# BurnhamG/PyTorch-ScalableFHVAE

Measured on AMD Instinct MI355X. Metric: segments/sec + ELBO (nats/frame), (B,20,80) fbank, higher is better.
Workload: dtype bf16; 1 GPU; c3: fhvae.FHVAE 2x256 LSTM enc/dec, z1=z2=32, 28k-seq mu2 table, batch 2048; per-GPU batch 2048, T=20, F=80, full train step (fwd+loss+bwd+Adam), intended objective, mu_idx uniform; global_batch=2048, parallelism=single

## Files before the change

pytorch-scalablefhvae_amd/csrc/lstm_fwd_wr.hip:

```cpp
#include <cstdlib>
#include <type_traits>

#include "lstm_cluster_dev.h"

#include "trace.h"

namespace fh {

constexpr int kFwH = 256, kFwG = 4 * kFwH, kFwHU = 32, kFwNU = 8, kFwThreads = 512;
typedef void __attribute__((address_space(3))) * fw_lds_p;

template <int NP>
__device__ __forceinline__ void fw_h_offsets(unsigned (&voff)[NP], int r0, int rlast, int piece0, int lane) {
#pragma unroll
  for (int i = 0; i < NP; ++i) {
    const int rw = (piece0 + i) * 2 + (lane >> 5), rg = r0 + rw;
    voff[i] = (unsigned)(rg < rlast ? rg : rlast) * (kFwH * 2) + (unsigned)(((lane & 31) ^ (rw & 15)) << 4);
  }
}
template <int NP>
__device__ __forceinline__ void fw_dma_h(char* img, __amdgpu_buffer_rsrc_t rs, const unsigned (&voff)[NP], unsigned slab_bytes, int piece0) {
#pragma unroll
  for (int i = 0; i < NP; ++i)
    __builtin_amdgcn_raw_ptr_buffer_load_lds(rs, (fw_lds_p)(img + (piece0 + i) * 1024), 16, voff[i], slab_bytes, 0, kSc1);
}
template <int NP>
__device__ __forceinline__ void fw_x_offsets(unsigned (&voff)[NP], int I, int r0, int rlast, int piece0, int lane) {
#pragma unroll
  for (int i = 0; i < NP; ++i) {
    const int rw = (piece0 + i) * 4 + (lane >> 4), rg = r0 + rw;
    voff[i] = (unsigned)(rg < rlast ? rg : rlast) * (unsigned)(I * 2) + (unsigned)(((lane & 15) ^ (rw & 15)) << 4);
  }
}
template <int NP>
__device__ __forceinline__ void fw_dma_x(char* img, __amdgpu_buffer_rsrc_t rs, const unsigned (&voff)[NP], unsigned slab_bytes, int nchx, int piece0,
                                         int lane) {
#pragma unroll
  for (int i = 0; i < NP; ++i) {
    const int rw = (piece0 + i) * 4 + (lane >> 4);
    if (((lane & 15) ^ (rw & 15)) < nchx)
      __builtin_amdgcn_raw_ptr_buffer_load_lds(rs, (fw_lds_p)(img + (piece0 + i) * 1024), 16, voff[i], slab_bytes, 0, 0);
  }
}
template <int NP>
__device__ __forceinline__ void fw_dma_xc(char* img, const u16* xc, int Ic, const u16* pad, int nchx, int r0, int rlast, int piece0, int lane) {
  const int nchc = Ic >> 3;
#pragma unroll
  for (int i = 0; i < NP; ++i) {
    const int rw = (piece0 + i) * 4 + (lane >> 4), rg = r0 + rw;
    const int64_t rc = rg < rlast ? rg : rlast;
    const int c = (lane & 15) ^ (rw & 15);
    if (c >= nchx) {
      const u16* src = c < nchx + nchc ? xc + rc * Ic + (c - nchx) * 8 : pad;
      __builtin_amdgcn_global_load_lds((const void __attribute__((address_space(1)))*)src, (fw_lds_p)(img + (piece0 + i) * 1024), 16, 0, 0);
    }
  }
}

template <int RT, int PDT = 4>
__global__ __launch_bounds__(kFwThreads) void lstm_fwd_wr_kernel(ClFwd p) {
  constexpr bool kSave = true;
#include "lstm_fwd_wr_body.h"
}
template <int RT, int PDT = 4>
__global__ __launch_bounds__(kFwThreads) void lstm_fwd_wr_infer_kernel(ClFwd p) {
  constexpr bool kSave = false;
#include "lstm_fwd_wr_body.h"
}

template __global__ void lstm_fwd_wr_kernel<2>(ClFwd);
template __global__ void lstm_fwd_wr_kernel<4>(ClFwd);
template __global__ void lstm_fwd_wr_infer_kernel<2>(ClFwd);
template __global__ void lstm_fwd_wr_infer_kernel<4>(ClFwd);

int cluster_fwd_wr(const ClFwd& p, hipStream_t st) {
  if ((int64_t)2 * p.T * p.B * kFwH * 2 >= (1LL << 31) || (int64_t)p.T * p.B * p.I * 2 >= (1LL << 31)) return FHVAE_ERR_LIMIT;
  if (p.NU != kFwNU || p.Mc > 64 || p.Mc % 16 != 0 || p.pre || p.K0 != p.I + p.Ic || p.K0 <= 0 || p.K0 > 128 || (p.I % 8) || (p.Ic % 8) ||
      (p.I > 0 && !p.x) || (p.Ic > 0 && !p.xcv))
    return FHVAE_ERR_SHAPE;
  const bool save = p.gates != nullptr;
  if (p.Mc <= 32 && save)
    hipLaunchKernelGGL((lstm_fwd_wr_kernel<2>), dim3(kGrid), dim3(kFwThreads), 0, st, p);
  else if (save)
    hipLaunchKernelGGL((lstm_fwd_wr_kernel<4>), dim3(kGrid), dim3(kFwThreads), 0, st, p);
  else if (p.Mc <= 32)
    hipLaunchKernelGGL((lstm_fwd_wr_infer_kernel<2>), dim3(kGrid), dim3(kFwThreads), 0, st, p);
  else
    hipLaunchKernelGGL((lstm_fwd_wr_infer_kernel<4>), dim3(kGrid), dim3(kFwThreads), 0, st, p);
  return fh_launch_status();
}

}
```

pytorch-scalablefhvae_amd/csrc/lstm_fwd_wr_body.h:

```cpp
  constexpr int H = kFwH, G = kFwG;
  constexpr int ROWS = RT * 16;
  __shared__ __attribute__((aligned(1024))) char img_h0[ROWS * 512];
  __shared__ __attribute__((aligned(1024))) char img_x[ROWS * 256];
  __shared__ __attribute__((aligned(1024))) char img_h1[ROWS * 512];
  constexpr int kGS = 272, kCS = 144, kHS = 80;
  constexpr int kStageL = ROWS * (kGS + 2 * kCS);
  __shared__ __attribute__((aligned(16))) char stage_all[2 * kStageL];
  __shared__ __attribute__((aligned(16))) char h16_all[ROWS * kHS];
  __shared__ int misc[2];
  const int tid = threadIdx.x, lane = tid & 63, wave = tid >> 6;
  const int r = lane & 15, q = lane >> 4;

  const int joined = cluster_join(p.sync, misc);
  if (joined < 0) return;
  const int info = joined & 255;
  const unsigned ep0 = (unsigned)(joined >> 8) * kSeqEpochs;
  const int cluster = (info >> 5) * (32 / kFwNU) + (info & 31) / kFwNU, me = (info & 31) % kFwNU;
  const int r0 = p.row0 + cluster * p.Mc;
  const int rend = min(p.row0 + p.nrows, r0 + p.Mc);
  if (r0 >= rend) return;
  unsigned* flags = p.sync + kSyncFlags + cluster * 32;
  unsigned* flagsB = flags + 8;
  const int B = p.B, T = p.T;
  const int um = me * kFwHU;
  const int ul = wave * 4 + q;
  if (tid == 0) misc[1] = 0;
  const int wv = __builtin_amdgcn_readfirstlane(wave);
  __syncthreads();

  const int wrow = (r & 3) * H + um + wave * 4 + (r >> 2);
  bf16x8 w_hh0[8], w_ih1[8], w_hh1[8], w_x[4];
#pragma unroll
  for (int ks = 0; ks < 8; ++ks) {
    const int64_t o = (int64_t)wrow * H + ks * 32 + q * 8;
    w_hh0[ks] = __builtin_bit_cast(bf16x8, *(const uint4*)(p.w_hh[0] + o));
    w_ih1[ks] = __builtin_bit_cast(bf16x8, *(const uint4*)(p.w_ih[1] + o));
    w_hh1[ks] = __builtin_bit_cast(bf16x8, *(const uint4*)(p.w_hh[1] + o));
  }
  const int nch0 = p.K0 / 8, nkx = (p.K0 + 31) / 32;
#pragma unroll
  for (int j = 0; j < 4; ++j) {
    const int c = j * 4 + q;
    uint4 v = uint4{0u, 0u, 0u, 0u};
    if (c < nch0) v = *(const uint4*)(p.w_ih0 + (int64_t)wrow * p.K0 + c * 8);
    w_x[j] = __builtin_bit_cast(bf16x8, v);
  }
  f32x4 add0, add1;
#pragma unroll
  for (int g = 0; g < 4; ++g) {
    add0[g] = p.b_ih[0][g * H + um + ul] + p.b_hh[0][g * H + um + ul];
    add1[g] = p.b_ih[1][g * H + um + ul] + p.b_hh[1][g * H + um + ul];
  }
  int hbase[4], xbase[4];
#pragma unroll
  for (int k3 = 0; k3 < 4; ++k3) {
    hbase[k3] = r * 512 + (((k3 * 4 + q) ^ r) << 4);
    xbase[k3] = r * 256 + (((k3 * 4 + q) ^ r) << 4);
  }
  float creg[2][RT];
#pragma unroll
  for (int l = 0; l < 2; ++l)
#pragma unroll
    for (int rt = 0; rt < RT; ++rt) creg[l][rt] = 0.f;
  unsigned long long* tl = (p.tlog && cluster == 0 && me == 0) ? p.tlog : nullptr;
  const bool xvar = p.I > 0;
  constexpr int NPX = RT * 4 / 4, NPH = RT * 8 / 4;
  const int nchx = p.I >> 3;
  const __amdgpu_buffer_rsrc_t hs_rs = make_rsrc(p.hs);
  const __amdgpu_buffer_rsrc_t x_rs = make_rsrc(xvar ? p.x : p.hs);
  unsigned voff_h[NPH], voff_x[NPX];
  fw_h_offsets<NPH>(voff_h, r0, rend - 1, (wv & 3) * NPH, lane);
  fw_x_offsets<NPX>(voff_x, p.I, r0, rend - 1, (wv & 3) * NPX, lane);
  const unsigned slab_h = (unsigned)B * (kFwH * 2), slab_x = (unsigned)B * (unsigned)(p.I * 2);
  if (wv < 4) {
    fw_dma_xc<NPX>(img_x, p.xcv, p.Ic, xvar ? p.x : p.xcv, nchx, r0, rend - 1, wv * NPX, lane);
    if (xvar) fw_dma_x<NPX>(img_x, x_rs, voff_x, 0u, nchx, wv * NPX, lane);
  }

  auto tail_stores = [&](int sp, int l, int wbase) {
    if (wv < wbase || wv >= wbase + 4) return;
    const int tq = tid - wbase * 64;
    const int t = sp - l;
    if (t < 0 || t >= T) return;
    const int64_t lt = (int64_t)l * T + t;
    const char* st = stage_all + l * kStageL;
    if constexpr (kSave) {
#pragma unroll
      for (int i = 0; i < ROWS * 16 / 256; ++i) {
        const int c = i * 256 + tq, rw = c >> 4, part = c & 15;
        const uint4 v = *(const uint4*)(st + rw * kGS + part * 16);
        if (r0 + rw < rend) *(uint4*)(p.gates + (lt * B + r0 + rw) * G + um * 4 + part * 8) = v;
      }
    }
    const bool top = l == 1 && p.hs_top_f32, last = p.hn && t == T - 1;
#pragma unroll
    for (int i = 0; i < ROWS * 8 / 256; ++i) {
      const int c = i * 256 + tq, rw = c >> 3, part = c & 7;
      if constexpr (kSave) {
        const uint4 v = *(const uint4*)(st + ROWS * kGS + rw * kCS + part * 16);
        if (r0 + rw < rend) *(uint4*)(p.cs + (lt * B + r0 + rw) * H + um + part * 4) = v;
      }
      if (top || last) {
        const uint4 hv = *(const uint4*)(st + ROWS * (kGS + kCS) + rw * kCS + part * 16);
        if (r0 + rw < rend) {
          if (top) *(uint4*)(p.hs_top_f32 + ((int64_t)t * B + r0 + rw) * H + um + part * 4) = hv;
          if (last) {
            *(uint4*)(p.hn + (int64_t)(r0 + rw) * (2 * H) + l * H + um + part * 4) = hv;
            if (p.hn_lp) {
              const float4 hf = __builtin_bit_cast(float4, hv);
              *(uint2*)(p.hn_lp + (int64_t)(r0 + rw) * (2 * H) + l * H + um + part * 4) = pack4(f32x4{hf.x, hf.y, hf.z, hf.w});
            }
          }
        }
      }
    }
  };
  auto h_out = [&](int l, int t, unsigned* fl, unsigned epoch, bool publish) {
    asm volatile("s_waitcnt lgkmcnt(0)\n\ts_barrier" ::: "memory");
    if (tid < ROWS * 4) {
      const int rw = tid >> 2, part = tid & 3;
      const uint4 v = *(const uint4*)(h16_all + rw * kHS + part * 16);
      if (r0 + rw < rend) *(uint4*)(p.hs + (((int64_t)l * T + t) * B + r0 + rw) * H + um + part * 8) = v;
    }
    if (publish) {
      if (wv < 4) asm volatile("s_waitcnt vmcnt(0)" ::: "memory");
      __syncthreads();
      if (tid == 0) __hip_atomic_store(fl + me, epoch, RLX_AGENT);
    } else {
      __syncthreads();
    }
  };
  auto flags_peek = [&](const unsigned* fl) -> unsigned {
    unsigned v = 0xffffffffu;
    if (lane < kFwNU) v = __hip_atomic_load(fl + lane, RLX_AGENT);
    return v;
  };
  auto flags_ready = [&](unsigned peeked, const unsigned* fl, unsigned epoch) -> bool {
    if (__all(peeked >= epoch)) return true;
    return cluster_wait(p.sync, fl, kFwNU, epoch);
  };
  unsigned peekA = 0u, peekB = 0u;

  constexpr int NI = 8 * RT;
  for (int s = 0; s <= T; ++s) {
    CL_TLOG(s * 8 + 0);
    const bool act0 = s < T, act1 = s >= 1;
    f32x4 acc[2][RT];
#pragma unroll
    for (int l = 0; l < 2; ++l)
#pragma unroll
      for (int rt = 0; rt < RT; ++rt) acc[l][rt] = f32x4{0.f, 0.f, 0.f, 0.f};
    if (wv < 4) asm volatile("s_waitcnt vmcnt(0)" ::: "memory");
    asm volatile("s_barrier" ::: "memory");
    if (misc[1]) return;
    CL_TLOG(s * 8 + 1);
    if (wv >= 4 && s >= 2) peekB = flags_peek(flagsB);
    if (s > 0) tail_stores(s - 1, 1, 0);
    auto mm = [&](auto l_c, const char* img, const bf16x8 (&w)[8], bool peek_a = false) {
      constexpr int l = decltype(l_c)::value;
      constexpr int PD = PDT;
      bf16x8 fb[PD + 1];
      auto frag = [&](int i) {
        const int ks = i / RT, rt = i % RT;
        fb[i % (PD + 1)] = __builtin_bit_cast(bf16x8, *(const uint4*)(img + hbase[ks & 3] + (ks >> 2) * 256 + rt * 8192));
      };
#pragma unroll
      for (int i = 0; i < PD; ++i) frag(i);
      if (PD > 2) __builtin_amdgcn_sched_barrier(0);
#pragma unroll
      for (int i = 0; i < NI; ++i) {
        const int ks = i / RT, rt = i % RT;
        if (i + PD < NI) frag(i + PD);
        if (PD > 2) __builtin_amdgcn_sched_barrier(0);
        acc[l][rt] = __builtin_amdgcn_mfma_f32_16x16x32_bf16(w[ks], fb[i % (PD + 1)], acc[l][rt], 0, 0, 0);
        if (PD > 2) __builtin_amdgcn_sched_barrier(0);
        if (i == NI - 1 && peek_a) peekA = flags_peek(flags);
      }
    };
    if (act0) {
#pragma unroll
      for (int j = 0; j < 4; ++j) {
        if (j >= nkx) break;
        bf16x8 b[RT];
#pragma unroll
        for (int rt = 0; rt < RT; ++rt) b[rt] = __builtin_bit_cast(bf16x8, *(const uint4*)(img_x + xbase[j] + rt * 4096));
        __builtin_amdgcn_sched_barrier(0);
#pragma unroll
        for (int rt = 0; rt < RT; ++rt) acc[0][rt] = __builtin_amdgcn_mfma_f32_16x16x32_bf16(w_x[j], b[rt], acc[0][rt], 0, 0, 0);
        __builtin_amdgcn_sched_barrier(0);
      }
      if (s > 0) mm(std::integral_constant<int, 0>{}, img_h0, w_hh0);
    }
    if (wv >= 4 && s >= 2) {
      if (!flags_ready(peekB, flagsB, ep0 + (unsigned)(s - 1))) {
        if (lane == 0) misc[1] = 1;
      } else {
        fw_dma_h<NPH>(img_h1, hs_rs, voff_h, (unsigned)(T + s - 2) * slab_h, (wv - 4) * NPH);
      }
    }
    CL_TLOG(s * 8 + 2);
    auto cell = [&](auto l_c, int rt) {
      constexpr int l = decltype(l_c)::value;
      const f32x4 v = acc[l][rt] + (l == 0 ? add0 : add1);
      const float ig = sigmoidf_(v[0]), fg = sigmoidf_(v[1]), gg = tanhf_(v[2]), og = sigmoidf_(v[3]);
      const float c = __builtin_fmaf(fg, creg[l][rt], ig * gg);
      const float h = og * tanhf_(c);
      creg[l][rt] = c;
      char* st = stage_all + l * kStageL;
      const int row = rt * 16 + r;
      if constexpr (kSave) {
        *(uint2*)(st + row * kGS + ul * 8) = pack4(f32x4{ig, fg, gg, og});
        *(float*)(st + ROWS * kGS + row * kCS + ul * 4) = c;
      }
      *(float*)(st + ROWS * (kGS + kCS) + row * kCS + ul * 4) = h;
      *(u16*)(h16_all + row * kHS + ul * 2) = f2bf(h);
    };
    if (s > 0) asm volatile("s_waitcnt lgkmcnt(0)\n\ts_barrier" ::: "memory");
    if (act0) {
#pragma unroll
      for (int rt = 0; rt < RT; ++rt) cell(std::integral_constant<int, 0>{}, rt);
      CL_TLOG(s * 8 + 3);
      h_out(0, s, flags, ep0 + (unsigned)(s + 1), true);
    }
    CL_TLOG(s * 8 + 4);
    if (act1) {
      mm(std::integral_constant<int, 1>{}, img_h0, w_ih1, wv < 4 && act0);
      if (wv >= 4) asm volatile("s_waitcnt vmcnt(0)" ::: "memory");
      asm volatile("s_waitcnt lgkmcnt(0)\n\ts_barrier" ::: "memory");
    }
    CL_TLOG(s * 8 + 5);
    auto request_a = [&]() {
      if (!flags_ready(act1 ? peekA : 0u, flags, ep0 + (unsigned)(s + 1))) {
        if (lane == 0) misc[1] = 1;
      } else {
        fw_dma_h<NPH>(img_h0, hs_rs, voff_h, (unsigned)s * slab_h, wv * NPH);
        if (xvar && s + 1 < T) fw_dma_x<NPX>(img_x, x_rs, voff_x, (unsigned)(s + 1) * slab_x, nchx, wv * NPX, lane);
      }
    };
    if (wv < 4 && act0 && !act1) request_a();
    if (act0) tail_stores(s, 0, 4);
    CL_TLOG(s * 8 + 6);
    if (act1) {
      if (s > 1) mm(std::integral_constant<int, 1>{}, img_h1, w_hh1);
      if (wv < 4 && act0) request_a();
#pragma unroll
      for (int rt = 0; rt < RT; ++rt) cell(std::integral_constant<int, 1>{}, rt);
      h_out(1, s - 1, flagsB, ep0 + (unsigned)s, s < T);
    }
    CL_TLOG(s * 8 + 7);
  }
  __syncthreads();
  tail_stores(T, 1, 0);
```

Baseline: 1.249 million segments/s.

## Halve LSTM forward block to 256 threads, each wave owning two unit tiles

```diff
diff --git a/pytorch-scalablefhvae_amd/csrc/lstm_fwd_wr.hip b/pytorch-scalablefhvae_amd/csrc/lstm_fwd_wr.hip
--- a/pytorch-scalablefhvae_amd/csrc/lstm_fwd_wr.hip
+++ b/pytorch-scalablefhvae_amd/csrc/lstm_fwd_wr.hip
@@ -7,7 +7,7 @@
 
 namespace fh {
 
-constexpr int kFwH = 256, kFwG = 4 * kFwH, kFwHU = 32, kFwNU = 8, kFwThreads = 512;
+constexpr int kFwH = 256, kFwG = 4 * kFwH, kFwHU = 32, kFwNU = 8, kFwThreads = 256;
 typedef void __attribute__((address_space(3))) * fw_lds_p;
 
 template <int NP>
@@ -58,12 +58,12 @@
 }
 
 template <int RT, int PDT = 4>
-__global__ __launch_bounds__(kFwThreads) void lstm_fwd_wr_kernel(ClFwd p) {
+__global__ __launch_bounds__(kFwThreads) __attribute__((amdgpu_waves_per_eu(1, 1))) void lstm_fwd_wr_kernel(ClFwd p) {
   constexpr bool kSave = true;
 #include "lstm_fwd_wr_body.h"
 }
 template <int RT, int PDT = 4>
-__global__ __launch_bounds__(kFwThreads) void lstm_fwd_wr_infer_kernel(ClFwd p) {
+__global__ __launch_bounds__(kFwThreads) __attribute__((amdgpu_waves_per_eu(1, 1))) void lstm_fwd_wr_infer_kernel(ClFwd p) {
   constexpr bool kSave = false;
 #include "lstm_fwd_wr_body.h"
 }
diff --git a/pytorch-scalablefhvae_amd/csrc/lstm_fwd_wr_body.h b/pytorch-scalablefhvae_amd/csrc/lstm_fwd_wr_body.h
--- a/pytorch-scalablefhvae_amd/csrc/lstm_fwd_wr_body.h
+++ b/pytorch-scalablefhvae_amd/csrc/lstm_fwd_wr_body.h
@@ -23,62 +23,82 @@
   unsigned* flagsB = flags + 8;
   const int B = p.B, T = p.T;
   const int um = me * kFwHU;
-  const int ul = wave * 4 + q;
+  const int ul0 = wave * 8 + q;
   if (tid == 0) misc[1] = 0;
   const int wv = __builtin_amdgcn_readfirstlane(wave);
   __syncthreads();
 
-  const int wrow = (r & 3) * H + um + wave * 4 + (r >> 2);
-  bf16x8 w_hh0[8], w_ih1[8], w_hh1[8], w_x[4];
-#pragma unroll
-  for (int ks = 0; ks < 8; ++ks) {
-    const int64_t o = (int64_t)wrow * H + ks * 32 + q * 8;
-    w_hh0[ks] = __builtin_bit_cast(bf16x8, *(const uint4*)(p.w_hh[0] + o));
-    w_ih1[ks] = __builtin_bit_cast(bf16x8, *(const uint4*)(p.w_ih[1] + o));
-    w_hh1[ks] = __builtin_bit_cast(bf16x8, *(const uint4*)(p.w_hh[1] + o));
-  }
+  bf16x8 w_hh0[2][8], w_ih1[2][8], w_hh1[2][8], w_x[2][4];
   const int nch0 = p.K0 / 8, nkx = (p.K0 + 31) / 32;
 #pragma unroll
-  for (int j = 0; j < 4; ++j) {
-    const int c = j * 4 + q;
-    uint4 v = uint4{0u, 0u, 0u, 0u};
-    if (c < nch0) v = *(const uint4*)(p.w_ih0 + (int64_t)wrow * p.K0 + c * 8);
-    w_x[j] = __builtin_bit_cast(bf16x8, v);
-  }
-  f32x4 add0, add1;
-#pragma unroll
-  for (int g = 0; g < 4; ++g) {
-    add0[g] = p.b_ih[0][g * H + um + ul] + p.b_hh[0][g * H + um + ul];
-    add1[g] = p.b_ih[1][g * H + um + ul] + p.b_hh[1][g * H + um + ul];
-  }
+  for (int tt = 0; tt < 2; ++tt) {
+    const int wrow = (r & 3) * H + um + wave * 8 + tt * 4 + (r >> 2);
+#pragma unroll
+    for (int ks = 0; ks < 8; ++ks) {
+      const int64_t o = (int64_t)wrow * H + ks * 32 + q * 8;
+      w_hh0[tt][ks] = __builtin_bit_cast(bf16x8, *(const uint4*)(p.w_hh[0] + o));
+      w_ih1[tt][ks] = __builtin_bit_cast(bf16x8, *(const uint4*)(p.w_ih[1] + o));
+      w_hh1[tt][ks] = __builtin_bit_cast(bf16x8, *(const uint4*)(p.w_hh[1] + o));
+    }
+#pragma unroll
+    for (int j = 0; j < 4; ++j) {
+      const int c = j * 4 + q;
+      uint4 v = uint4{0u, 0u, 0u, 0u};
+      if (c < nch0) v = *(const uint4*)(p.w_ih0 + (int64_t)wrow * p.K0 + c * 8);
+      w_x[tt][j] = __builtin_bit_cast(bf16x8, v);
+    }
+  }
+#pragma unroll
+  for (int tt = 0; tt < 2; ++tt) {
+#pragma unroll
+    for (int ks = 0; ks < 8; ++ks) {
+      asm volatile("" : "+a"(w_hh0[tt][ks]));
+      asm volatile("" : "+a"(w_ih1[tt][ks]));
+      asm volatile("" : "+a"(w_hh1[tt][ks]));
+    }
+#pragma unroll
+    for (int j = 0; j < 4; ++j) asm volatile("" : "+a"(w_x[tt][j]));
+  }
+  f32x4 add0[2], add1[2];
+#pragma unroll
+  for (int tt = 0; tt < 2; ++tt)
+#pragma unroll
+    for (int g = 0; g < 4; ++g) {
+      const int u = g * H + um + ul0 + tt * 4;
+      add0[tt][g] = p.b_ih[0][u] + p.b_hh[0][u];
+      add1[tt][g] = p.b_ih[1][u] + p.b_hh[1][u];
+    }
   int hbase[4], xbase[4];
 #pragma unroll
   for (int k3 = 0; k3 < 4; ++k3) {
     hbase[k3] = r * 512 + (((k3 * 4 + q) ^ r) << 4);
     xbase[k3] = r * 256 + (((k3 * 4 + q) ^ r) << 4);
   }
-  float creg[2][RT];
-#pragma unroll
-  for (int l = 0; l < 2; ++l)
-#pragma unroll
-    for (int rt = 0; rt < RT; ++rt) creg[l][rt] = 0.f;
+  float creg[2][2][RT];
+#pragma unroll
+  for (int tt = 0; tt < 2; ++tt)
+#pragma unroll
+    for (int l = 0; l < 2; ++l)
+#pragma unroll
+      for (int rt = 0; rt < RT; ++rt) creg[tt][l][rt] = 0.f;
   unsigned long long* tl = (p.tlog && cluster == 0 && me == 0) ? p.tlog : nullptr;
   const bool xvar = p.I > 0;
-  constexpr int NPX = RT * 4 / 4, NPH = RT * 8 / 4;
+  constexpr int NPX = RT * 4 / 2, NPH = RT * 8 / 2;
   const int nchx = p.I >> 3;
   const __amdgpu_buffer_rsrc_t hs_rs = make_rsrc(p.hs);
   const __amdgpu_buffer_rsrc_t x_rs = make_rsrc(xvar ? p.x : p.hs);
   unsigned voff_h[NPH], voff_x[NPX];
-  fw_h_offsets<NPH>(voff_h, r0, rend - 1, (wv & 3) * NPH, lane);
-  fw_x_offsets<NPX>(voff_x, p.I, r0, rend - 1, (wv & 3) * NPX, lane);
+  fw_h_offsets<NPH>(voff_h, r0, rend - 1, (wv & 1) * NPH, lane);
+  fw_x_offsets<NPX>(voff_x, p.I, r0, rend - 1, (wv & 1) * NPX, lane);
   const unsigned slab_h = (unsigned)B * (kFwH * 2), slab_x = (unsigned)B * (unsigned)(p.I * 2);
-  if (wv < 4) {
+  if (wv < 2) {
     fw_dma_xc<NPX>(img_x, p.xcv, p.Ic, xvar ? p.x : p.xcv, nchx, r0, rend - 1, wv * NPX, lane);
     if (xvar) fw_dma_x<NPX>(img_x, x_rs, voff_x, 0u, nchx, wv * NPX, lane);
   }
 
+  constexpr int NH = kFwThreads / 2;
   auto tail_stores = [&](int sp, int l, int wbase) {
-    if (wv < wbase || wv >= wbase + 4) return;
+    if (wv < wbase || wv >= wbase + 2) return;
     const int tq = tid - wbase * 64;
     const int t = sp - l;
     if (t < 0 || t >= T) return;
@@ -86,16 +106,16 @@
     const char* st = stage_all + l * kStageL;
     if constexpr (kSave) {
 #pragma unroll
-      for (int i = 0; i < ROWS * 16 / 256; ++i) {
-        const int c = i * 256 + tq, rw = c >> 4, part = c & 15;
+      for (int i = 0; i < ROWS * 16 / NH; ++i) {
+        const int c = i * NH + tq, rw = c >> 4, part = c & 15;
         const uint4 v = *(const uint4*)(st + rw * kGS + part * 16);
         if (r0 + rw < rend) *(uint4*)(p.gates + (lt * B + r0 + rw) * G + um * 4 + part * 8) = v;
       }
     }
     const bool top = l == 1 && p.hs_top_f32, last = p.hn && t == T - 1;
 #pragma unroll
-    for (int i = 0; i < ROWS * 8 / 256; ++i) {
-      const int c = i * 256 + tq, rw = c >> 3, part = c & 7;
+    for (int i = 0; i < ROWS * 8 / NH; ++i) {
+      const int c = i * NH + tq, rw = c >> 3, part = c & 7;
       if constexpr (kSave) {
         const uint4 v = *(const uint4*)(st + ROWS * kGS + rw * kCS + part * 16);
         if (r0 + rw < rend) *(uint4*)(p.cs + (lt * B + r0 + rw) * H + um + part * 4) = v;
@@ -117,13 +137,16 @@
   };
   auto h_out = [&](int l, int t, unsigned* fl, unsigned epoch, bool publish) {
     asm volatile("s_waitcnt lgkmcnt(0)\n\ts_barrier" ::: "memory");
-    if (tid < ROWS * 4) {
-      const int rw = tid >> 2, part = tid & 3;
-      const uint4 v = *(const uint4*)(h16_all + rw * kHS + part * 16);
-      if (r0 + rw < rend) *(uint4*)(p.hs + (((int64_t)l * T + t) * B + r0 + rw) * H + um + part * 8) = v;
+    if (wv < 2) {
+#pragma unroll
+      for (int i = 0; i < ROWS * 4 / NH; ++i) {
+        const int c = i * NH + tid, rw = c >> 2, part = c & 3;
+        const uint4 v = *(const uint4*)(h16_all + rw * kHS + part * 16);
+        if (r0 + rw < rend) *(uint4*)(p.hs + (((int64_t)l * T + t) * B + r0 + rw) * H + um + part * 8) = v;
+      }
     }
     if (publish) {
-      if (wv < 4) asm volatile("s_waitcnt vmcnt(0)" ::: "memory");
+      if (wv < 2) asm volatile("s_waitcnt vmcnt(0)" ::: "memory");
       __syncthreads();
       if (tid == 0) __hip_atomic_store(fl + me, epoch, RLX_AGENT);
     } else {
@@ -145,18 +168,20 @@
   for (int s = 0; s <= T; ++s) {
     CL_TLOG(s * 8 + 0);
     const bool act0 = s < T, act1 = s >= 1;
-    f32x4 acc[2][RT];
-#pragma unroll
-    for (int l = 0; l < 2; ++l)
-#pragma unroll
-      for (int rt = 0; rt < RT; ++rt) acc[l][rt] = f32x4{0.f, 0.f, 0.f, 0.f};
-    if (wv < 4) asm volatile("s_waitcnt vmcnt(0)" ::: "memory");
+    f32x4 acc[2][2][RT];
+#pragma unroll
+    for (int tt = 0; tt < 2; ++tt)
+#pragma unroll
+      for (int l = 0; l < 2; ++l)
+#pragma unroll
+        for (int rt = 0; rt < RT; ++rt) acc[tt][l][rt] = f32x4{0.f, 0.f, 0.f, 0.f};
+    if (wv < 2) asm volatile("s_waitcnt vmcnt(0)" ::: "memory");
     asm volatile("s_barrier" ::: "memory");
     if (misc[1]) return;
     CL_TLOG(s * 8 + 1);
-    if (wv >= 4 && s >= 2) peekB = flags_peek(flagsB);
+    if (wv >= 2 && s >= 2) peekB = flags_peek(flagsB);
     if (s > 0) tail_stores(s - 1, 1, 0);
-    auto mm = [&](auto l_c, const char* img, const bf16x8 (&w)[8], bool peek_a = false) {
+    auto mm = [&](auto l_c, const char* img, const bf16x8 (&w)[2][8], bool peek_a = false) {
       constexpr int l = decltype(l_c)::value;
       constexpr int PD = PDT;
       bf16x8 fb[PD + 1];
@@ -172,7 +197,8 @@
         const int ks = i / RT, rt = i % RT;
         if (i + PD < NI) frag(i + PD);
         if (PD > 2) __builtin_amdgcn_sched_barrier(0);
-        acc[l][rt] = __builtin_amdgcn_mfma_f32_16x16x32_bf16(w[ks], fb[i % (PD + 1)], acc[l][rt], 0, 0, 0);
+        acc[0][l][rt] = __builtin_amdgcn_mfma_f32_16x16x32_bf16(w[0][ks], fb[i % (PD + 1)], acc[0][l][rt], 0, 0, 0);
+        acc[1][l][rt] = __builtin_amdgcn_mfma_f32_16x16x32_bf16(w[1][ks], fb[i % (PD + 1)], acc[1][l][rt], 0, 0, 0);
         if (PD > 2) __builtin_amdgcn_sched_barrier(0);
         if (i == NI - 1 && peek_a) peekA = flags_peek(flags);
       }
@@ -186,34 +212,46 @@
         for (int rt = 0; rt < RT; ++rt) b[rt] = __builtin_bit_cast(bf16x8, *(const uint4*)(img_x + xbase[j] + rt * 4096));
         __builtin_amdgcn_sched_barrier(0);
 #pragma unroll
-        for (int rt = 0; rt < RT; ++rt) acc[0][rt] = __builtin_amdgcn_mfma_f32_16x16x32_bf16(w_x[j], b[rt], acc[0][rt], 0, 0, 0);
+        for (int rt = 0; rt < RT; ++rt) {
+          acc[0][0][rt] = __builtin_amdgcn_mfma_f32_16x16x32_bf16(w_x[0][j], b[rt], acc[0][0][rt], 0, 0, 0);
+          acc[1][0][rt] = __builtin_amdgcn_mfma_f32_16x16x32_bf16(w_x[1][j], b[rt], acc[1][0][rt], 0, 0, 0);
+        }
         __builtin_amdgcn_sched_barrier(0);
       }
       if (s > 0) mm(std::integral_constant<int, 0>{}, img_h0, w_hh0);
     }
-    if (wv >= 4 && s >= 2) {
+    if (wv >= 2 && s >= 2) {
       if (!flags_ready(peekB, flagsB, ep0 + (unsigned)(s - 1))) {
         if (lane == 0) misc[1] = 1;
       } else {
-        fw_dma_h<NPH>(img_h1, hs_rs, voff_h, (unsigned)(T + s - 2) * slab_h, (wv - 4) * NPH);
+        fw_dma_h<NPH>(img_h1, hs_rs, voff_h, (unsigned)(T + s - 2) * slab_h, (wv - 2) * NPH);
       }
     }
     CL_TLOG(s * 8 + 2);
+    const bool hf32[2] = {p.hn && s == T - 1, p.hs_top_f32 || (p.hn && s == T)};
     auto cell = [&](auto l_c, int rt) {
       constexpr int l = decltype(l_c)::value;
-      const f32x4 v = acc[l][rt] + (l == 0 ? add0 : add1);
-      const float ig = sigmoidf_(v[0]), fg = sigmoidf_(v[1]), gg = tanhf_(v[2]), og = sigmoidf_(v[3]);
-      const float c = __builtin_fmaf(fg, creg[l][rt], ig * gg);
-      const float h = og * tanhf_(c);
-      creg[l][rt] = c;
       char* st = stage_all + l * kStageL;
       const int row = rt * 16 + r;
-      if constexpr (kSave) {
-        *(uint2*)(st + row * kGS + ul * 8) = pack4(f32x4{ig, fg, gg, og});
-        *(float*)(st + ROWS * kGS + row * kCS + ul * 4) = c;
-      }
-      *(float*)(st + ROWS * (kGS + kCS) + row * kCS + ul * 4) = h;
-      *(u16*)(h16_all + row * kHS + ul * 2) = f2bf(h);
+      float h[2];
+#pragma unroll
+      for (int tt = 0; tt < 2; ++tt) {
+        const int ul = ul0 + tt * 4;
+        const f32x4 v = acc[tt][l][rt] + (l == 0 ? add0[tt] : add1[tt]);
+        const float ig = sigmoidf_(v[0]), fg = sigmoidf_(v[1]), gg = tanhf_(v[2]), og = sigmoidf_(v[3]);
+        const float c = __builtin_fmaf(fg, creg[tt][l][rt], ig * gg);
+        h[tt] = og * tanhf_(c);
+        creg[tt][l][rt] = c;
+        if constexpr (kSave) {
+          *(uint2*)(st + row * kGS + ul * 8) = pack4(f32x4{ig, fg, gg, og});
+          *(float*)(st + ROWS * kGS + row * kCS + ul * 4) = c;
+        }
+        *(u16*)(h16_all + row * kHS + ul * 2) = f2bf(h[tt]);
+      }
+      if (hf32[l]) {
+        *(float*)(st + ROWS * (kGS + kCS) + row * kCS + ul0 * 4) = h[0];
+        *(float*)(st + ROWS * (kGS + kCS) + row * kCS + (ul0 + 4) * 4) = h[1];
+      }
     };
     if (s > 0) asm volatile("s_waitcnt lgkmcnt(0)\n\ts_barrier" ::: "memory");
     if (act0) {
@@ -224,8 +262,8 @@
     }
     CL_TLOG(s * 8 + 4);
     if (act1) {
-      mm(std::integral_constant<int, 1>{}, img_h0, w_ih1, wv < 4 && act0);
-      if (wv >= 4) asm volatile("s_waitcnt vmcnt(0)" ::: "memory");
+      mm(std::integral_constant<int, 1>{}, img_h0, w_ih1, wv < 2 && act0);
+      if (wv >= 2) asm volatile("s_waitcnt vmcnt(0)" ::: "memory");
       asm volatile("s_waitcnt lgkmcnt(0)\n\ts_barrier" ::: "memory");
     }
     CL_TLOG(s * 8 + 5);
@@ -237,12 +275,12 @@
         if (xvar && s + 1 < T) fw_dma_x<NPX>(img_x, x_rs, voff_x, (unsigned)(s + 1) * slab_x, nchx, wv * NPX, lane);
       }
     };
-    if (wv < 4 && act0 && !act1) request_a();
-    if (act0) tail_stores(s, 0, 4);
+    if (wv < 2 && act0 && !act1) request_a();
+    if (act0) tail_stores(s, 0, 2);
     CL_TLOG(s * 8 + 6);
     if (act1) {
       if (s > 1) mm(std::integral_constant<int, 1>{}, img_h1, w_hh1);
-      if (wv < 4 && act0) request_a();
+      if (wv < 2 && act0) request_a();
 #pragma unroll
       for (int rt = 0; rt < RT; ++rt) cell(std::integral_constant<int, 1>{}, rt);
       h_out(1, s - 1, flagsB, ep0 + (unsigned)s, s < T);
```

Measured after the change: 1.197 million segments/s. -4.2%, worse.
